# oleg-savchenko/jax_nbody_emulator_with_dj

Measured on AMD Instinct MI355X. Metric: voxels/sec (disp+vel) on 512^3 box, ndiv=4, higher is better.
Workload: dtype f32-equivalent: f16x3 split MFMA (3 f16 MFMAs per product, f32 accumulate)

## Files before the change

### jax_nbody_emulator_with_dj_amd/csrc/nbe_kernels_wino.h

```cpp

#ifndef NBE_EPI_MAX
#define NBE_EPI_MAX 1
#endif
#ifndef NBE_WINO_ZROW
#define NBE_WINO_ZROW 1
#endif
#ifndef NBE_WINO_ITEMREG
#define NBE_WINO_ITEMREG 1
#endif
#ifndef NBE_WINO_LOU
#define NBE_WINO_LOU (NBE_XF_F32 ? 0 : 1)
#endif
constexpr int NBE_MAX_WSTAGES = 32;
constexpr int NBE_MAX_WSKIP = 16;
constexpr float WINO_WSCALE = 16384.0f;
constexpr float WINO_WSCALE_F16 = 256.0f;

struct WinoSrc { const char* xa; const char* xb; long dxd; const char* w; long psb; float sb; int pad_; };

struct WinoKArgs {
    int H, W, Dv, Hv, Wv, Ho, Wo;
    int nchunk, cout_groups, flags, ntiles, tny, tnx;
    int zblock;
    float* y; float* dy; long out_pstride; int out_g0;
    const float* bias; const float* gout; const float* beta;
    const float* r; const float* dr; long res_pstride;
    float inv_scale;
    int nskip;
    long dws_delta;
    WinoSrc st[NBE_MAX_WSTAGES + NBE_MAX_WSKIP];
};

template <bool SKIP, bool NOVEL, bool F16 = false>
__global__ __launch_bounds__(512, 2) void conv_h3w_kernel(WinoKArgs a) {
    static_assert(!(F16 && NOVEL), "the float16 form has no displacement-only variant");
    typedef HGGeom<false> G;
    constexpr int NW = 8, CT = 64, TAPU = G::TAPU, WGU = G::WG, XBASE = G::XBASE, MT = 4, NT = 2, NTILE = 8;
    constexpr int ZROW = G::LDS_UNITS;
    f32x4* lds = lds_h3;
    const half8* L8 = (const half8*)lds_h3;
    half8* L8w = (half8*)lds_h3;
    const int tid = threadIdx.x;
    const int lane = tid & 63;
    const int wave = __builtin_amdgcn_readfirstlane(tid >> 6);
    const int c = lane & 15, q = lane >> 4, kh = q & 1, ks = q >> 1;

    const int nct = (a.cout_groups + 7) / 8;
    const int vt = xcd_tile(blockIdx.x, a.ntiles * nct);
    const int tile = vt / nct, ct = vt - tile * nct;
    const int npair = a.Dv >> 1;
    int zp, ty, tx;
    {
        const int zb = a.zblock;
        const int full = (npair / zb) * zb;
        const int per_blk = zb * a.tny * a.tnx;
        if (tile < (npair / zb) * per_blk) {
            const int blk = tile / per_blk, r = tile - blk * per_blk;
            const int zi = r % zb, tyx = r / zb;
            zp = blk * zb + zi; ty = tyx / a.tnx; tx = tyx - ty * a.tnx;
        } else {
            const int r = tile - (npair / zb) * per_blk, rem = npair - full;
            const int zi = r % rem, tyx = r / rem;
            zp = full + zi; ty = tyx / a.tnx; tx = tyx - ty * a.tnx;
        }
    }
    const int y0 = ty * (NOVEL ? 2 * HP_ROWS : HP_ROWS), x0 = tx * HP_COLS, z0 = 2 * zp;
    const int nst = 4 * a.nchunk;

    const long to = (((long)z0 * a.H + y0) * a.W + x0) * 16;
    const long wcm = (long)ct * nst * WGU * 16, wcs = (long)ct * a.nskip * TAPU * 16;

    struct Nxt { const char *xa, *xb, *w0; long dxd, psb; float sb; } nx;
    auto set_next = [&](int s) {
        const WinoSrc e = a.st[s];
        nx.xa = e.xa + to; nx.xb = e.xb + to; nx.dxd = e.dxd; nx.psb = e.psb; nx.w0 = e.w + (SKIP && s >= nst ? wcs : wcm); nx.sb = e.sb;
    };
    unsigned lane16 = (unsigned)lane << 4;
    asm volatile("" : "+v"(lane16));
    auto dma_w = [&](int buf, int t) {
        const int n = wave + NW * t;
        unsigned l16 = (unsigned)lane;
        if (NBE_WINO_ZROW && !F16) l16 = lane16;
        else asm volatile("v_lshlrev_b32 %0, 4, %0" : "+v"(l16));
        if (n < G::NWI) dma16s(nx.w0 + (long)n * 1024, l16, lds + buf * WGU + n * 64);
    };
    auto dma_raw = [&](int buf) {
        unsigned l16 = (unsigned)lane;
        asm volatile("v_lshlrev_b32 %0, 4, %0" : "+v"(l16));
        dma16s(nx.w0 + (wave < 4 ? 0 : a.dws_delta) + (long)(wave & 3) * 1024, l16, lds + buf * WGU + wave * 64);
#pragma unroll
        for (int t = 0; t < 6; ++t) {
            const int tensor = t / 3, n = wave + NW * (t % 3), pl = n / 6, k = n - 6 * pl;
            const int u = k * 64 + lane;
            const int uu = u < HP_PL ? u : HP_PL - 1;
            const int row = (uu * 241) >> 13, col = uu - row * HP_RS;
            if (u < HP_PL)
                dma16s(nx.xa + (tensor ? nx.dxd : 0) + (long)pl * nx.psb, (unsigned)(row * a.W + col) * 16u,
                       lds + XBASE + buf * HQ_XB + tensor * HQ_XT + pl * HQ_PP + k * 64);
        }
    };
    constexpr bool ITEMREG = NBE_WINO_ITEMREG && !F16;
    int it_uu[3] = {0, 0, 0};
    unsigned it_go[3] = {0u, 0u, 0u};
    if (ITEMREG) {
#pragma unroll
        for (int j = 0; j < 3; ++j) {
            const int u = ((wave + NW * j) % 6) * 64 + lane;
            it_uu[j] = u < HP_PL ? u : HP_PL - 1;
            const int row = (it_uu[j] * 241) >> 13, col = it_uu[j] - row * HP_RS;
            it_go[j] = (unsigned)(row * a.W + col) * 16u;
        }
#pragma unroll
        for (int j = 0; j < 3; ++j) asm volatile("" : "+v"(it_uu[j]), "+v"(it_go[j]));
    }
    auto item_unit = [&](int j, bool& valid) {
        if (ITEMREG) {
            valid = lane < HP_PL - ((wave + NW * j) % 6) * 64;
            return it_uu[j];
        }
        int l = lane;
        asm volatile("" : "+v"(l));
        const int u = ((wave + NW * j) % 6) * 64 + l;
        valid = u < HP_PL;
        return valid ? u : HP_PL - 1;
    };
    auto item_goff_j = [&](int j) {
        if (ITEMREG) return it_go[j];
        bool v;
        const int uu = item_unit(j, v);
        const int row = (uu * 241) >> 13, col = uu - row * HP_RS;
        return (unsigned)(row * a.W + col) * 16u;
    };
    typedef unsigned int u32x4 __attribute__((ext_vector_type(4)));
    struct Stg { half8 ah, al, bh, bl; float sb; };
    auto st_load = [&](int j, Stg& g) {
        const int n = wave + NW * j;
        const long po = ((n / 12) ? nx.dxd : 0) + (long)(((n % 12) / 6) * 2) * nx.psb;
        const char* pa = nx.xa + po;
        const char* pb = nx.xb + po;
        const unsigned go = item_goff_j(j);
        const __amdgpu_buffer_rsrc_t ra = __builtin_amdgcn_make_buffer_rsrc((void*)pa, 0, 0xffffffffu, 0x00027000);
        const __amdgpu_buffer_rsrc_t rb = __builtin_amdgcn_make_buffer_rsrc((void*)pb, 0, 0xffffffffu, 0x00027000);
        const unsigned pso = (unsigned)nx.psb;
        auto ld = [&](half8& d, __amdgpu_buffer_rsrc_t r, unsigned so) {
            const u32x4 v = __builtin_amdgcn_raw_buffer_load_b128(r, go, so, 0);
            d = __builtin_bit_cast(half8, v);
        };
        ld(g.ah, ra, 0); ld(g.al, ra, pso); ld(g.bh, rb, 0); ld(g.bl, rb, pso);
        g.sb = nx.sb;
    };
#if NBE_XF_F32
    struct Xf { u32x4 HI, LO; float t0, t1; unsigned h; };
    auto xf_step = [&](const Stg& g, Xf& x, int k) {
        const int r = k >> 2, m = k & 3;
        const unsigned AH = __builtin_bit_cast(u32x4, g.ah)[r], AL = __builtin_bit_cast(u32x4, g.al)[r];
        const unsigned BH = __builtin_bit_cast(u32x4, g.bh)[r], BL = __builtin_bit_cast(u32x4, g.bl)[r];
        const float inv = H3_INV, sinv = g.sb * H3_INV, sb = g.sb, k2048 = H3_SCALE;
        if (m == 0) {
            asm("v_fma_mix_f32 %0, %1, %2, %3 op_sel:[0,0,0] op_sel_hi:[1,0,1]" : "=v"(x.t0) : "v"(AL), "s"(inv), "v"(AH));
            asm("v_fma_mix_f32 %0, %1, %2, %0 op_sel:[0,0,0] op_sel_hi:[1,0,0]" : "+v"(x.t0) : "v"(BL), "s"(sinv));
            asm("v_fma_mix_f32 %0, %1, %2, %0 op_sel:[0,0,0] op_sel_hi:[1,0,0]" : "+v"(x.t0) : "v"(BH), "s"(sb));
        } else if (m == 1) {
            asm("v_fma_mix_f32 %0, %1, %2, %3 op_sel:[1,0,1] op_sel_hi:[1,0,1]" : "=v"(x.t1) : "v"(AL), "s"(inv), "v"(AH));
            asm("v_fma_mix_f32 %0, %1, %2, %0 op_sel:[1,0,0] op_sel_hi:[1,0,0]" : "+v"(x.t1) : "v"(BL), "s"(sinv));
            asm("v_fma_mix_f32 %0, %1, %2, %0 op_sel:[1,0,0] op_sel_hi:[1,0,0]" : "+v"(x.t1) : "v"(BH), "s"(sb));
        } else if (m == 2) {
            asm("v_cvt_pk_f16_f32 %0, %1, %2" : "=v"(x.h) : "v"(x.t0), "v"(x.t1));
            asm("v_fma_mix_f32 %0, %1, -1.0, %0 op_sel:[0,0,0] op_sel_hi:[1,0,0]" : "+v"(x.t0) : "v"(x.h));
            asm("v_fma_mix_f32 %0, %1, -1.0, %0 op_sel:[1,0,0] op_sel_hi:[1,0,0]" : "+v"(x.t1) : "v"(x.h));
        } else {
            unsigned l;
            asm("v_fma_mixlo_f16 %0, %1, %2, 0 op_sel_hi:[0,0,0]" : "=v"(l) : "v"(x.t0), "s"(k2048));
            asm("v_fma_mixhi_f16 %0, %1, %2, 0 op_sel_hi:[0,0,0]" : "+v"(l) : "v"(x.t1), "s"(k2048));
            x.HI[r] = x.h; x.LO[r] = l;
        }
    };
#else
    struct Xf { u32x4 HI, LO; unsigned s, bb, e1, e2, l1; };
    auto xf_step = [&](const Stg& g, Xf& x, int k) {
        const int r = k >> 2, m = k & 3;
        const unsigned AH = __builtin_bit_cast(u32x4, g.ah)[r], AL = __builtin_bit_cast(u32x4, g.al)[r];
        const unsigned BH = __builtin_bit_cast(u32x4, g.bh)[r], BL = __builtin_bit_cast(u32x4, g.bl)[r];
        const unsigned sbp = g.sb < 0.f ? 0xBC00BC00u : 0x3C003C00u, k2048 = 0x68006800u;
        if (F16) {
            if (m == 0) asm("v_pk_fma_f16 %0, %1, %2, %3" : "=v"(x.s) : "v"(BH), "s"(sbp), "v"(AH));
            else if (m == 1) asm("v_pk_fma_f16 %0, %1, %2, %3" : "=v"(x.l1) : "v"(BL), "s"(sbp), "v"(AL));
            else if (m == 3) { x.HI[r] = x.s; x.LO[r] = x.l1; }
            (void)k2048;
        } else
        if (m == 0) {
            asm("v_pk_fma_f16 %0, %1, %2, %3" : "=v"(x.s) : "v"(BH), "s"(sbp), "v"(AH));
            asm("v_pk_add_f16 %0, %1, %2 neg_lo:[0,1] neg_hi:[0,1]" : "=v"(x.bb) : "v"(x.s), "v"(AH));
        } else if (m == 1) {
            asm("v_pk_add_f16 %0, %1, %2 neg_lo:[0,1] neg_hi:[0,1]" : "=v"(x.e1) : "v"(x.s), "v"(x.bb));
            asm("v_pk_fma_f16 %0, %1, %2, %3 neg_lo:[0,0,1] neg_hi:[0,0,1]" : "=v"(x.e2) : "v"(BH), "s"(sbp), "v"(x.bb));
        } else if (m == 2) {
            asm("v_pk_add_f16 %0, %1, %2 neg_lo:[0,1] neg_hi:[0,1]" : "=v"(x.e1) : "v"(AH), "v"(x.e1));
            asm("v_pk_fma_f16 %0, %1, %2, %3" : "=v"(x.l1) : "v"(BL), "s"(sbp), "v"(AL));
        } else {
            unsigned err, l;
            asm("v_pk_add_f16 %0, %1, %2" : "=v"(err) : "v"(x.e1), "v"(x.e2));
#if NBE_WINO_LOU
            const unsigned kinv = 0x10001000u;
            asm("v_pk_fma_f16 %0, %1, %2, %3" : "=v"(l) : "v"(x.l1), "s"(kinv), "v"(err));
            (void)k2048;
#else
            asm("v_pk_fma_f16 %0, %1, %2, %3" : "=v"(l) : "v"(err), "s"(k2048), "v"(x.l1));
#endif
            x.HI[r] = x.s; x.LO[r] = l;
        }
    };
#endif
    auto st_write = [&](int j, int buf, const Xf& x) {
        bool valid;
        const int n = wave + NW * j;
        const int lo_ = XBASE + buf * HQ_XB + (n / 12) * HQ_XT + (((n % 12) / 6) * 2) * HQ_PP + item_unit(j, valid);
        if (valid) {
            L8w[lo_] = __builtin_bit_cast(half8, x.HI);
            L8w[lo_ + HQ_PP] = __builtin_bit_cast(half8, x.LO);
        }
    };
    auto st_store = [&](int j, int buf, Stg& g) {
        Xf x;
#pragma unroll
        for (int k = 0; k < 16; ++k) xf_step(g, x, k);
        st_write(j, buf, x);
    };

    f32x4 YA[NTILE], DA[NTILE], YB[NTILE], DB[NTILE];
#pragma unroll
    for (int t = 0; t < NTILE; ++t)
#pragma unroll
        for (int e = 0; e < 4; ++e) { YA[t][e] = 0.f; DA[t][e] = 0.f; YB[t][e] = 0.f; DB[t][e] = 0.f; }
    auto mm = [&](f32x4& acc, const half8& A, const half8& B) {
        asm("v_mfma_f32_16x16x32_f16 %0, %1, %2, %0" : "+a"(acc) : "v"(A), "v"(B));
    };
    auto mmz = [&](f32x4& acc, const half8& A, const half8& B) {
        asm("s_nop 1\n\tv_mfma_f32_16x16x32_f16 %0, %1, %2, %0" : "+a"(acc) : "v"(A), "v"(B));
    };

    const int rowp = wave;
    const int aP = (ks * 4 + 2 * kh) * CT + c;
    const int bB = (2 * kh) * HQ_PP + rowp * HP_RS + c;
    const int bP1 = bB + ks, bP32 = bB + 32 * ks;
    auto LA = [&](half8 (&r)[MT], int idx) {
#pragma unroll
        for (int mt = 0; mt < MT; ++mt) r[mt] = L8[idx + 16 * mt];
    };
    auto LB = [&](half8 (&r)[NT], int idx) {
#pragma unroll
        for (int nt = 0; nt < NT; ++nt) r[nt] = L8[idx + 16 * nt];
    };
    const _Float16 kInv = (_Float16)H3_INV;
#define SNAKE(i) ((((i) >> 1) & 1) ? ((i) ^ 1) : (i))
    auto nohook = [](int) {};
    auto MM8h = [&](f32x4 (&acc)[NTILE], const half8 (&A)[MT], const half8 (&B)[NT], int slot, int nb, bool px, bool zsel,
                    bool hooked, auto&& hook) {
#pragma unroll
        for (int i = 0; i < NTILE; ++i) {
            const int t = SNAKE(i);
            if (zsel && (i % NT) == 0) mmz(acc[t], A[t / NT], B[t % NT]); else
            mm(acc[t], A[t / NT], B[t % NT]);
            if (hooked) { hook(i); __builtin_amdgcn_sched_barrier(0); }
            if (slot >= 0 && (i % 4) == 3) {
                if (px) dma_w(nb, slot + i / 4);
                __builtin_amdgcn_sched_barrier(0);
            }
        }
    };
    auto MM8 = [&](f32x4 (&acc)[NTILE], const half8 (&A)[MT], const half8 (&B)[NT], int slot, int nb, bool px, bool zsel = false) {
        MM8h(acc, A, B, slot, nb, px, zsel, false, nohook);
    };
    auto MM8s = [&](f32x4 (&acc)[NTILE], half8 (&P)[MT], const half8 (&A)[MT], const half8 (&B)[NT], int slot, int nb, bool px) {
        P[0] = A[0] * kInv;
#pragma unroll
        for (int i = 0; i < NTILE; ++i) {
            const int t = SNAKE(i);
            if ((i % NT) == 0) { if (t / NT + 1 < MT) P[t / NT + 1] = A[t / NT + 1] * kInv; mmz(acc[t], P[t / NT], B[t % NT]); }
            else mm(acc[t], P[t / NT], B[t % NT]);
            if (slot >= 0 && (i % 4) == 3) {
                if (px) dma_w(nb, slot + i / 4);
                __builtin_amdgcn_sched_barrier(0);
            }
        }
    };
#define NBE_SB __builtin_amdgcn_sched_barrier(0)
    half8 wh[MT], wl[MT], wp[MT], xh[NT], xl[NT], dxh[NT], dxl[NT];
    auto pair = [&](f32x4 (&Y)[NTILE], f32x4 (&DY)[NTILE], int slot0, int nb, bool px, int wa, int xp,
                    auto&& preXl, auto&& preW, auto&& preXh, auto&& mid, bool hooked, auto&& hook, auto&& after3) {
        if (F16) {
            LB(dxh, xp + HQ_XT); LA(wl, wa + CT + aP);
            NBE_SB; MM8h(Y, wh, xh, slot0, nb, px, false, hooked, [&](int t) { hook(t); }); NBE_SB;
            LB(dxl, xp + HQ_XT + HQ_PP);
            NBE_SB; MM8h(Y, wl, xl, slot0 < 0 ? -1 : slot0 + 2, nb, px, false, hooked, [&](int t) { hook(8 + t); }); NBE_SB;
            after3();
            mid();
            preXl(); preXh();
            NBE_SB; MM8(DY, wh, dxh, slot0 < 0 ? -1 : slot0 + 4, nb, px); NBE_SB;
            preW();
            NBE_SB; MM8(DY, wl, dxl, -1, nb, px); NBE_SB;
            return;
        }
        LB(dxh, xp + HQ_XT);
#if NBE_WINO_LOU
        NBE_SB; MM8(Y, wh, xl, slot0, nb, px); NBE_SB;
#else
        NBE_SB; MM8s(Y, wp, wh, xl, slot0, nb, px); NBE_SB;
#endif
        LB(dxl, xp + HQ_XT + HQ_PP);
        NBE_SB; MM8h(Y, wh, xh, slot0 < 0 ? -1 : slot0 + 2, nb, px, false, hooked, [&](int t) { hook(t); }); NBE_SB;
        LA(wl, wa + CT + aP);
        NBE_SB; MM8h(DY, wh, dxh, slot0 < 0 ? -1 : slot0 + 4, nb, px, false, hooked, [&](int t) { hook(8 + t); }); NBE_SB;
        after3();
        mid();
#if NBE_WINO_LOU
        NBE_SB; MM8(DY, wh, dxl, -1, nb, px); NBE_SB;
#else
        NBE_SB; MM8(DY, wp, dxl, -1, nb, px); NBE_SB;
#endif
        preXl(); preW();
        NBE_SB; MM8(Y, wl, xh, -1, nb, px); NBE_SB;
        preXh();
        NBE_SB; MM8(DY, wl, dxh, -1, nb, px); NBE_SB;
    };

    constexpr int SH4 = HP_RS + 1, SH5 = HP_RS + 2, SH7 = 2 * HP_RS + 1;
    auto stage = [&](f32x4 (&Y)[NTILE], f32x4 (&DY)[NTILE], int s, auto nxt) {
        constexpr int NXT = decltype(nxt)::value;
        constexpr bool px = NXT == 1;
        const bool pre = px && s + 1 != 2 * a.nchunk;
        if (NXT) set_next(s + 1);
        int par = s & 1;
        asm volatile("" : "+s"(par));
        int nb = 1 - par;
        asm volatile("" : "+s"(nb));
        const int wb = par * WGU, xb = XBASE + par * HQ_XB;
        const int wbn = nb * WGU, xbn = XBASE + nb * HQ_XB;
        Stg g;
        Xf xf;
        auto hk = [&](int k) { xf_step(g, xf, k); };
        auto none = [] {};
        if (NXT == 2) dma_raw(nb);
        if (px) st_load(0, g);
        pair(Y, DY, 0, nb, px, wb, xb + bP1,
             [&] { LB(xl, xb + 2 + bP32 + HQ_PP); }, [&] { LA(wh, wb + 2 * TAPU + aP); }, [&] { LB(xh, xb + 2 + bP32); },
             none, false, nohook, none);
        half8 a1[MT], a2[MT], b1x[NT], b1d[NT];
        const int aS = wb + 4 * TAPU + (2 * kh + (F16 ? ks : 0)) * CT + c;
        const int bS = xb + (2 * kh + ks) * HQ_PP + rowp * HP_RS + c + SH4;
        pair(Y, DY, -1, nb, px, wb + 2 * TAPU, xb + 2 + bP32,
             [&] { LB(b1x, bS); }, [&] { LA(a1, aS); }, [&] { LB(b1d, bS + HQ_XT); }, none,
             px, hk, [&] { if (px) { st_write(0, nb, xf); st_load(1, g); } });
        const half8 zero = {0, 0, 0, 0, 0, 0, 0, 0};
        if (F16) {
            NBE_SB; MM8(Y, a1, b1x, -1, 0, false); NBE_SB;
            LB(xl, xb + SH5 + bP32 + HQ_PP); LB(xh, xb + SH5 + bP32); LA(wh, wb + 5 * TAPU + aP);
            NBE_SB; MM8(DY, a1, b1d, -1, 0, false); NBE_SB;
        } else {
#if NBE_WINO_LOU
        NBE_SB; MM8(Y, a1, b1x, -1, 0, false); NBE_SB;
#else
        {
            const _Float16 m1 = ks ? kInv : (_Float16)1.0f;
#pragma unroll
            for (int mt = 0; mt < MT; ++mt) a1[mt] = a1[mt] * m1;
        }
        NBE_SB; MM8(Y, a1, b1x, -1, 0, false, true); NBE_SB;
#endif
#if NBE_WINO_ZROW
        LA(a2, ks ? ZROW + c : aS + CT);
#else
        LA(a2, aS + CT);
#endif
        LB(xl, xb + SH5 + bP32 + HQ_PP);
        NBE_SB; MM8(DY, a1, b1d, -1, 0, false); NBE_SB;
        LB(xh, xb + SH5 + bP32); LA(wh, wb + 5 * TAPU + aP);
#if NBE_WINO_ZROW
        NBE_SB; MM8(Y, a2, b1x, -1, 0, false); NBE_SB;
#else
#pragma unroll
        for (int mt = 0; mt < MT; ++mt) a2[mt] = ks ? zero : a2[mt];
        NBE_SB; MM8(Y, a2, b1x, -1, 0, false, true); NBE_SB;
#endif
        MM8(DY, a2, b1d, -1, 0, false); NBE_SB;
        }
        pair(Y, DY, -1, nb, px, wb + 5 * TAPU, xb + SH5 + bP32,
             [&] { LB(xl, xb + SH7 + bP1 + HQ_PP); }, [&] { LA(wh, wb + 7 * TAPU + aP); }, [&] { LB(xh, xb + SH7 + bP1); },
             none, px, hk, [&] { if (px) { st_write(1, nb, xf); st_load(2, g); } });
        pair(Y, DY, -1, nb, px, wb + 7 * TAPU, xb + SH7 + bP1,
             [&] { if (pre) LB(xl, xbn + bP1 + HQ_PP); }, [&] { if (pre) LA(wh, wbn + aP); }, [&] { if (pre) LB(xh, xbn + bP1); },
             [&] { asm volatile("s_waitcnt vmcnt(0) lgkmcnt(0)\n\ts_barrier" ::: "memory"); },
             px, hk, [&] { if (px) st_write(2, nb, xf); });
    };

    auto raw_stage = [&](f32x4 (&Y)[NTILE], f32x4 (&DY)[NTILE], int s, bool px) {
        if (px) set_next(s + 1);
        int par = s & 1;
        asm volatile("" : "+s"(par));
        int nb = 1 - par;
        asm volatile("" : "+s"(nb));
        const int wb = par * WGU, xb = XBASE + par * HQ_XB;
        if (px) dma_raw(nb);
        half8 a1[MT], a2[MT], d1[MT], d2[MT], bx[NT], bd[NT];
        const half8 zero = {0, 0, 0, 0, 0, 0, 0, 0};
        const _Float16 m1 = ks ? kInv : (_Float16)1.0f;
        const int aS = wb + (2 * kh) * CT + c;
        const int bS = xb + (2 * kh + ks) * HQ_PP + rowp * HP_RS + c + SH4;
        if (F16) {
            const int aF = wb + (2 * kh + ks) * CT + c;
            LA(a1, aF); LB(bx, bS); LB(bd, bS + HQ_XT); LA(d1, aF + TAPU);
            NBE_SB; MM8(Y, a1, bx, -1, 0, false); NBE_SB;
            MM8(DY, a1, bd, -1, 0, false); NBE_SB;
            MM8(DY, d1, bx, -1, 0, false); NBE_SB;
            asm volatile("s_waitcnt vmcnt(0) lgkmcnt(0)\n\ts_barrier" ::: "memory");
            return;
        }
        LA(a1, aS); LB(bx, bS); LA(a2, aS + CT); LB(bd, bS + HQ_XT);
#pragma unroll
        for (int mt = 0; mt < MT; ++mt) a1[mt] = a1[mt] * m1;
        NBE_SB; MM8(Y, a1, bx, -1, 0, false, true); NBE_SB;
        if (!NOVEL) LA(d1, aS + TAPU);
#pragma unroll
        for (int mt = 0; mt < MT; ++mt) a2[mt] = ks ? zero : a2[mt];
        NBE_SB; MM8(Y, a2, bx, -1, 0, false, true); NBE_SB;
        if (!NOVEL) LA(d2, aS + TAPU + CT);
        if (NOVEL || !(a.flags & F_SKIP_NODX)) {
            NBE_SB; MM8(DY, a1, bd, -1, 0, false); NBE_SB;
            MM8(DY, a2, bd, -1, 0, false); NBE_SB;
        }
        if (!NOVEL) {
#pragma unroll
            for (int mt = 0; mt < MT; ++mt) { d1[mt] = d1[mt] * m1; d2[mt] = ks ? zero : d2[mt]; }
            NBE_SB; MM8(DY, d1, bx, -1, 0, false, true); NBE_SB;
            MM8(DY, d2, bx, -1, 0, false, true); NBE_SB;
        }
        asm volatile("s_waitcnt vmcnt(0) lgkmcnt(0)\n\ts_barrier" ::: "memory");
    };

    {
        if (NBE_WINO_ZROW && !F16 && tid < 64) L8w[ZROW + tid] = half8{0, 0, 0, 0, 0, 0, 0, 0};
        set_next(0);
#pragma unroll
        for (int k = 0; k < G::NWS; ++k) dma_w(0, k);
        {
            Stg g0, g1, g2;
            st_load(0, g0); st_load(1, g1); st_load(2, g2);
            st_store(0, 0, g0); st_store(1, 0, g1); st_store(2, 0, g2);
        }
        asm volatile("s_waitcnt vmcnt(0) lgkmcnt(0)" ::: "memory");
        __syncthreads();
        LA(wh, aP); LB(xl, XBASE + bP1 + HQ_PP); LB(xh, XBASE + bP1);
    }

    auto butterfly = [&] {
            asm volatile("s_nop 15\n\ts_nop 15" ::: "memory");
#pragma unroll
            for (int t = 0; t < NTILE; ++t) {
                f32x4 p, m;
#pragma unroll
                for (int e = 0; e < 4; ++e) { p[e] = acc_read(YA[t][e]); m[e] = acc_read(YB[t][e]); }
                YA[t] = p + m; YB[t] = p - m;
                asm volatile("" : "+a"(YA[t]), "+a"(YB[t]));
                __builtin_amdgcn_sched_barrier(0);
#pragma unroll
                for (int e = 0; e < 4; ++e) { p[e] = acc_read(DA[t][e]); m[e] = acc_read(DB[t][e]); }
                DA[t] = p + m; DB[t] = p - m;
                asm volatile("" : "+a"(DA[t]), "+a"(DB[t]));
                __builtin_amdgcn_sched_barrier(0);
            }
            asm volatile("s_nop 7" ::: "memory");
            LA(wh, aP); LB(xl, XBASE + bP1 + HQ_PP); LB(xh, XBASE + bP1);
    };
    const int npairs = 2 * a.nchunk;
    for (int s2 = 0; s2 + 1 < npairs; ++s2) {
        if (s2 == a.nchunk) butterfly();
        stage(YA, DA, 2 * s2, std::integral_constant<int, 1>());
        stage(YB, DB, 2 * s2 + 1, std::integral_constant<int, 1>());
    }
    if (npairs - 1 == a.nchunk) butterfly();
    stage(YA, DA, 2 * npairs - 2, std::integral_constant<int, 1>());
    stage(YB, DB, 2 * npairs - 1, std::integral_constant<int, SKIP ? 2 : 0>());
    if (SKIP) {
        for (int sc = 0; sc < a.nskip; ++sc) {
            raw_stage(YA, DA, nst + 2 * sc, true);
            raw_stage(YB, DB, nst + 2 * sc + 1, sc + 1 < a.nskip);
        }
    }
#undef NBE_SB
#undef SNAKE
    asm volatile("s_nop 15\n\ts_nop 15" ::: "memory");

    const bool act = a.flags & F_ACT, gauge = !NOVEL && a.gout != nullptr;
    f32x4 bv[MT], be[MT], gv[MT];
    int unit[MT];
    bool uok[MT];
#pragma unroll
    for (int mt = 0; mt < MT; ++mt) {
        unit[mt] = ct * (CT / 8) + 2 * mt + ks;
        uok[mt] = unit[mt] < a.cout_groups;
        if (!uok[mt]) unit[mt] = a.cout_groups - 1;
        bv[mt] = *(const f32x4*)(a.bias + unit[mt] * 8 + 4 * kh);
        be[mt] = f32x4{0.f, 0.f, 0.f, 0.f};
        if (!NOVEL) be[mt] = *(const f32x4*)(a.beta + unit[mt] * 8 + 4 * kh);
        gv[mt] = f32x4{0.f, 0.f, 0.f, 0.f};
        if (!NOVEL && gauge) gv[mt] = *(const f32x4*)(a.gout + unit[mt] * 8 + 4 * kh);
    }
#pragma unroll
    for (int mt = 0; mt < MT; ++mt) asm volatile("" : "+v"(bv[mt]), "+v"(be[mt]), "+v"(gv[mt]));
    long ob_mt[MT];
#pragma unroll
    for (int mt = 0; mt < MT; ++mt) ob_mt[mt] = (long)(a.out_g0 + (F16 ? 1 : 2) * unit[mt]) * a.out_pstride * 16 + 8 * kh;
    const long ol_off = a.out_pstride * 16;
    auto epilogue = [&](f32x4 (&Y)[NTILE], f32x4 (&DY)[NTILE], int z) {
        int o[NT];
        bool ook[NT], ook2[NT];
#pragma unroll
        for (int nt = 0; nt < NT; ++nt) {
            const int yy = y0 + rowp, xx = x0 + 16 * nt + c;
            ook[nt] = yy < a.Hv && xx < a.Wv;
            ook2[nt] = NOVEL && yy + HP_ROWS < a.Hv && xx < a.Wv;
            o[nt] = ook[nt] ? (z * a.Ho + yy) * a.Wo + xx : z * a.Ho * a.Wo;
        }
        half4 r0[F16 ? NTILE : 1], r1[F16 ? NTILE : 1];
        const bool res = F16 && (a.flags & F_RES);
        if (F16 && res) {
#pragma unroll
            for (int t = 0; t < NTILE; ++t) {
                const int mt = t / NT, nt = t % NT;
                const long rb = ((long)unit[mt] * a.res_pstride + (long)o[nt]) * 16 + 8 * kh;
                r0[t] = *(const half4*)((const char*)a.r + rb);
                r1[t] = *(const half4*)((const char*)a.dr + rb);
            }
#pragma unroll
            for (int t = 0; t < NTILE; ++t) asm volatile("" : "+v"(r0[t]), "+v"(r1[t]));
        }
#pragma unroll
        for (int mt = 0; mt < MT; ++mt) {
#pragma unroll
            for (int nt = 0; nt < NT; ++nt) {
                const int t = mt * NT + nt;
                f32x4 v, dv;
                __builtin_amdgcn_sched_barrier(0);
#pragma unroll
                for (int e = 0; e < 4; ++e) {
                    const float yp = acc_read(Y[t][e]) * a.inv_scale;
                    v[e] = yp + bv[mt][e];
                    dv[e] = acc_read(DY[t][e]) * a.inv_scale + be[mt][e] * yp;
                }
                if (F16 && res) {
#pragma unroll
                    for (int e = 0; e < 4; ++e) { v[e] += (float)r0[t][e]; dv[e] += (float)r1[t][e]; }
                }
                if (act) {
#pragma unroll
                    for (int e = 0; e < 4; ++e) {
                        dv[e] = v[e] > 0.f ? dv[e] : 0.01f * dv[e];
                        v[e] = (F16 || !NBE_EPI_MAX) ? (v[e] >= 0.f ? v[e] : 0.01f * v[e]) : __builtin_fmaxf(v[e], 0.01f * v[e]);
                    }
                }
                if (gauge) {
#pragma unroll
                    for (int e = 0; e < 4; ++e) dv[e] += gv[mt][e] * v[e];
                }
                if (F16) {
                    if (uok[mt] && ook[nt]) {
                        const long ob = ob_mt[mt] + (long)o[nt] * 16;
                        half4 h, dh;
#pragma unroll
                        for (int e = 0; e < 4; ++e) { h[e] = (_Float16)v[e]; dh[e] = (_Float16)dv[e]; }
                        *(half4*)((char*)a.y + ob) = h;
                        *(half4*)((char*)a.dy + ob) = dh;
                    }
                } else
                if (NOVEL) {
#pragma unroll
                    for (int e = 0; e < 4; ++e) {
                        dv[e] = acc_read(DY[t][e]) * a.inv_scale + bv[mt][e];
                        if (act) dv[e] = dv[e] >= 0.f ? dv[e] : 0.01f * dv[e];
                    }
                    const long ob = ob_mt[mt] + (long)o[nt] * 16;
                    const long ol = ob + ol_off;
                    const long r8 = (long)HP_ROWS * a.Wo * 16;
                    half4 hi, lo;
                    if (uok[mt] && ook[nt]) {
                        split4(v, hi, lo);
                        *(half4*)((char*)a.y + ob) = hi;
                        *(half4*)((char*)a.y + ol) = lo;
                    }
                    if (uok[mt] && ook2[nt]) {
                        split4(dv, hi, lo);
                        *(half4*)((char*)a.y + ob + r8) = hi;
                        *(half4*)((char*)a.y + ol + r8) = lo;
                    }
                } else
                if (uok[mt] && ook[nt]) {
                    const long ob = ob_mt[mt] + (long)o[nt] * 16;
                    const long ol = ob + ol_off;
                    half4 hi, lo;
                    split4(v, hi, lo);
                    *(half4*)((char*)a.y + ob) = hi;
                    *(half4*)((char*)a.y + ol) = lo;
                    split4(dv, hi, lo);
                    *(half4*)((char*)a.dy + ob) = hi;
                    *(half4*)((char*)a.dy + ol) = lo;
                }
            }
        }
    };
    epilogue(YA, DA, z0);
    epilogue(YB, DB, z0 + 1);
}

__global__ __launch_bounds__(256) void pack_h3w_kernel(const float* __restrict__ w, int cout, int cin, int nchunk, long total,
                                                       _Float16* __restrict__ dst, int* __restrict__ flag, int f16) {
    const long idx = (long)blockIdx.x * blockDim.x + threadIdx.x;
    if (idx >= total) return;
    long r = idx;
    const int j = (int)(r % 8); r /= 8;
    const int co = (int)(r % 64); r /= 64;
    const int u = (int)(r % 4); r /= 4;
    const int tap = (int)(r % 9); r /= 9;
    const int stage = (int)(r % (4 * nchunk)); r /= 4 * nchunk;
    const int ct = (int)r;
    const int chunk = stage >> 2, xi = stage & 3;
    const int h = u >> 1, part = u & 1;
    const int ci = f16 ? chunk * 32 + 8 * u + j : chunk * 16 + 8 * h + j, oc = ct * 64 + co;
    float v = 0.f;
    if (oc < cout && ci < cin) {
        const float* p = w + (((size_t)oc * cin + ci) * 3) * 9 + tap;
        const float w0 = p[0], w1 = p[9], w2 = p[18];
        v = xi == 0 ? w0 : xi == 1 ? 0.5f * (w0 + w1 + w2) : xi == 2 ? 0.5f * (w0 - w1 + w2) : -w2;
    }
    v *= f16 ? WINO_WSCALE_F16 : WINO_WSCALE;
    if (!(fabsf(v) <= 60000.f)) { atomicOr(flag, 1); v = 0.f; }
    const _Float16 hi = (_Float16)v;
    dst[idx] = (part == 0 || f16) ? hi : (_Float16)(v - (float)hi);
}

void launch_pack_h3w(const float* w_oidhw, int cout, int cin, int cin_pad, int ctiles, float* dst, int* flag, hipStream_t s, int prec) {
    const bool f16 = prec == PREC_F16;
    const int nchunk = cin_pad / (f16 ? 32 : 16);
    const long total = (long)ctiles * 4 * nchunk * 9 * 4 * 64 * 8;
    hipLaunchKernelGGL(pack_h3w_kernel, dim3((unsigned)((total + 255) / 256)), dim3(256), 0, s, w_oidhw, cout, cin, nchunk, total,
                       (_Float16*)dst, flag, f16 ? 1 : 0);
}

static int launch_h3w(const ConvKArgs& ka_in, const float* ww, const float* wws, long wws_set_floats, int ctiles, hipStream_t s,
                      bool novel = false, bool f16 = false) {
    typedef HGGeom<false> G;
    constexpr size_t smem = (size_t)(G::LDS_UNITS + 64) * 16;
    static_assert(smem <= 160 * 1024, "LDS budget of one CU");
    ConvKArgs ka = ka_in;
    if (f16) {
        if (novel || (ka.nchunk & 1) || (ka.csplit < ka.nchunk && (ka.csplit & 1))) return 1;
        if (ka.nskip > 0 && ((ka.nskip & 1) || (ka.s_csplit < ka.nskip && (ka.s_csplit & 1)) || (ka.flags & F_SKIP_NODX))) return 1;
        ka.nchunk /= 2; if (ka.csplit < (1 << 29)) ka.csplit /= 2;
        ka.nskip /= 2; if (ka.s_csplit < (1 << 29)) ka.s_csplit /= 2;
    }
    if (!ww || (!f16 && (ka.flags & F_RES)) || (ka.Dv & 1) || 4 * ka.nchunk > NBE_MAX_WSTAGES || (!novel && !ka.beta)) return 1;
    if (ka.nskip > 0 && (!wws || 2 * ka.nskip > NBE_MAX_WSKIP)) return 1;
    if (ctiles != (ka.cout_groups + 7) / 8) return 1;
    if (std::max(ka.in_pstride, ka.csplit < ka.nchunk ? ka.in2_pstride : 0L) * 16 + 16L * (HP_ROWS + 2) * ka.W >= (1L << 32) - (1L << 20)) return 1;
    WinoKArgs wa;
    wa.H = ka.H; wa.W = ka.W; wa.Dv = ka.Dv; wa.Hv = ka.Hv; wa.Wv = ka.Wv; wa.Ho = ka.Ho; wa.Wo = ka.Wo;
    wa.nchunk = ka.nchunk; wa.cout_groups = ka.cout_groups; wa.flags = ka.flags;
    const int trows = novel ? 2 * HP_ROWS : HP_ROWS;
    wa.tny = (ka.Hv + trows - 1) / trows;
    wa.tnx = (ka.Wv + HP_COLS - 1) / HP_COLS;
    wa.ntiles = (ka.Dv / 2) * wa.tny * wa.tnx;
    wa.y = ka.y; wa.dy = ka.dy; wa.out_pstride = ka.out_pstride; wa.out_g0 = ka.out_g0;
    wa.bias = ka.bias; wa.gout = novel ? nullptr : ka.gout; wa.beta = novel ? nullptr : ka.beta;
    const long rows8 = (long)HP_ROWS * ka.W * 16;
    wa.inv_scale = 1.0f / (f16 ? WINO_WSCALE_F16 : WINO_WSCALE);
    wa.r = ka.r; wa.dr = ka.dr; wa.res_pstride = ka.res_pstride;
    wa.zblock = std::min(8, ka.Dv / 2);
    wa.nskip = ka.nskip; wa.dws_delta = wws_set_floats * 4;
    static const int XI[2][2] = {{1, 2}, {0, 3}};
    static const int PA[4] = {0, 1, 2, 1}, PB[4] = {2, 2, 1, 3};
    static const float SB[4] = {-1.f, 1.f, -1.f, -1.f};
    const long plane = (long)ka.H * ka.W * 16;
    for (int ph = 0; ph < 2; ++ph)
        for (int chunk = 0; chunk < ka.nchunk; ++chunk)
            for (int ab = 0; ab < 2; ++ab) {
                const int xi = XI[ph][ab];
                const bool second = chunk >= ka.csplit;
                const long ps = second ? ka.in2_pstride : ka.in_pstride;
                const char* x = (const char*)(second ? ka.x2 : ka.x);
                const char* dx = (const char*)(second ? ka.dx2 : ka.dx);
                const long off = (long)(second ? chunk - ka.csplit : chunk) * 4 * ps * 16;
                WinoSrc& e = wa.st[(ph * ka.nchunk + chunk) * 2 + ab];
                e.xa = x + off + PA[xi] * plane; e.xb = x + off + PB[xi] * plane; e.dxd = novel ? rows8 : dx - x;
                e.w = (const char*)ww + (long)(chunk * 4 + xi) * G::WG * 16; e.psb = ps * 16; e.sb = SB[xi]; e.pad_ = 0;
            }
    for (int sc = 0; sc < ka.nskip; ++sc)
        for (int ab = 0; ab < 2; ++ab) {
            const bool second = sc >= ka.s_csplit;
            const long ps = second ? ka.s2_pstride : ka.s_pstride;
            const char* x = (const char*)(second ? ka.xs2 : ka.xs);
            const char* dx = (const char*)(second ? ka.dxs2 : ka.dxs);
            const long off = (long)(second ? sc - ka.s_csplit : sc) * 4 * ps * 16 + ab * plane;
            WinoSrc& e = wa.st[4 * ka.nchunk + 2 * sc + ab];
            e.xa = x + off; e.xb = e.xa; e.dxd = novel ? rows8 : dx - x; e.w = (const char*)wws + (long)sc * G::TAPU * 16; e.psb = ps * 16; e.sb = 0.f; e.pad_ = 0;
        }
    const bool skip = ka.nskip > 0;
    if (novel) wa.dws_delta = 0;
    auto kern = f16 ? (skip ? conv_h3w_kernel<true, false, true> : conv_h3w_kernel<false, false, true>)
              : novel ? (skip ? conv_h3w_kernel<true, true> : conv_h3w_kernel<false, true>)
              : (skip ? conv_h3w_kernel<true, false> : conv_h3w_kernel<false, false>);
    ensure_lds_limit((const void*)kern, smem);
    dim3 grid(wa.ntiles * ctiles, 1, 1), block(512, 1, 1);
    hipLaunchKernelGGL(kern, grid, block, smem, s, wa);
    return 0;
}
```

Measured before the change: 97.89 million.

## Preload all skip weights to LDS and stream skip activations via registers

For the non-F16 skip path, the kernel now DMAs every skip chunk's weights into the idle LDS buffers in one go at the last main stage. Skip-input activations are loaded straight from global memory into registers with double buffering, replacing the per-stage LDS staging and its barriers. The skip loop is restructured into raw_chunk, which processes YA and YB in the same pass and folds the scale into MFMA hooks. This aims to remove the per-skip-stage barrier and DMA round trips, but adds register pressure and global-load latency exposure, and limits the number of skip chunks to eight.

```diff
diff --git a/jax_nbody_emulator_with_dj_amd/csrc/nbe_kernels_wino.h b/jax_nbody_emulator_with_dj_amd/csrc/nbe_kernels_wino.h
--- a/jax_nbody_emulator_with_dj_amd/csrc/nbe_kernels_wino.h
+++ b/jax_nbody_emulator_with_dj_amd/csrc/nbe_kernels_wino.h
@@ -68,12 +68,17 @@
     const int nst = 4 * a.nchunk;
 
     const long to = (((long)z0 * a.H + y0) * a.W + x0) * 16;
-    const long wcm = (long)ct * nst * WGU * 16, wcs = (long)ct * a.nskip * TAPU * 16;
+    const long wcm = (long)ct * nst * WGU * 16;
+    auto wcs_of = [&] { return (long)ct * a.nskip * TAPU * 16; };
 
     struct Nxt { const char *xa, *xb, *w0; long dxd, psb; float sb; } nx;
     auto set_next = [&](int s) {
         const WinoSrc e = a.st[s];
-        nx.xa = e.xa + to; nx.xb = e.xb + to; nx.dxd = e.dxd; nx.psb = e.psb; nx.w0 = e.w + (SKIP && s >= nst ? wcs : wcm); nx.sb = e.sb;
+        nx.xa = e.xa + to; nx.xb = e.xb + to; nx.dxd = e.dxd; nx.psb = e.psb; nx.w0 = e.w + wcm; nx.sb = e.sb;
+    };
+    auto set_next_raw = [&](int s) {
+        const WinoSrc e = a.st[s];
+        nx.xa = e.xa + to; nx.xb = e.xb + to; nx.dxd = e.dxd; nx.psb = e.psb; nx.w0 = e.w + wcs_of(); nx.sb = e.sb;
     };
     unsigned lane16 = (unsigned)lane << 4;
     asm volatile("" : "+v"(lane16));
@@ -98,6 +103,16 @@
                 dma16s(nx.xa + (tensor ? nx.dxd : 0) + (long)pl * nx.psb, (unsigned)(row * a.W + col) * 16u,
                        lds + XBASE + buf * HQ_XB + tensor * HQ_XT + pl * HQ_PP + k * 64);
         }
+    };
+    constexpr int SKWU = 2 * TAPU;
+    static_assert(4 * SKWU <= WGU && 4 * SKWU <= HQ_XB && 2 * 8 <= NBE_MAX_WSKIP, "eight chunks of skip weights fit the idle buffers");
+    auto skw = [&](int buf, int sc) { return sc < 4 ? buf * WGU + sc * SKWU : XBASE + buf * HQ_XB + (sc - 4) * SKWU; };
+    auto dma_skipw = [&](int buf) {
+        unsigned l16 = (unsigned)lane;
+        asm volatile("v_lshlrev_b32 %0, 4, %0" : "+v"(l16));
+#pragma nounroll
+        for (int sc = 0; sc < a.nskip; ++sc)
+            dma16s(a.st[nst + 2 * sc].w + wcs_of() + (wave < 4 ? 0 : a.dws_delta) + (long)(wave & 3) * 1024, l16, lds + skw(buf, sc) + wave * 64);
     };
     constexpr bool ITEMREG = NBE_WINO_ITEMREG && !F16;
     int it_uu[3] = {0, 0, 0};
@@ -324,12 +339,34 @@
         NBE_SB; MM8(DY, wl, dxh, -1, nb, px); NBE_SB;
     };
 
+    struct RawB { half8 x[2][NT], d[2][NT]; };
+    RawB rb0, rb1;
+    const bool skdx = NOVEL || !(a.flags & F_SKIP_NODX);
+    auto raw_load = [&](int sc, RawB& b, bool on) {
+        int l = lane;
+        asm volatile("" : "+v"(l));
+        const unsigned vox = (unsigned)((wave + 1) * a.W + 1 + (l & 15)) * 16u;
+        const unsigned pl = (unsigned)(2 * ((l >> 4) & 1) + (l >> 5));
+#pragma unroll
+        for (int ab = 0; ab < 2; ++ab) {
+            const WinoSrc& e = a.st[nst + 2 * sc + ab];
+            const char* gx = e.xa + to + (on ? (long)pl * e.psb + vox : 0L);
+            const char* gd = gx + (skdx ? e.dxd : 0L);
+#pragma unroll
+            for (int nt = 0; nt < NT; ++nt) {
+                b.x[ab][nt] = *(const half8*)(gx + 256 * nt);
+                b.d[ab][nt] = *(const half8*)(gd + 256 * nt);
+            }
+        }
+    };
+
     constexpr int SH4 = HP_RS + 1, SH5 = HP_RS + 2, SH7 = 2 * HP_RS + 1;
     auto stage = [&](f32x4 (&Y)[NTILE], f32x4 (&DY)[NTILE], int s, auto nxt) {
         constexpr int NXT = decltype(nxt)::value;
         constexpr bool px = NXT == 1;
         const bool pre = px && s + 1 != 2 * a.nchunk;
-        if (NXT) set_next(s + 1);
+        if (NXT == 1) set_next(s + 1);
+        if (NXT == 2 && F16) set_next_raw(s + 1);
         int par = s & 1;
         asm volatile("" : "+s"(par));
         int nb = 1 - par;
@@ -340,7 +377,10 @@
         Xf xf;
         auto hk = [&](int k) { xf_step(g, xf, k); };
         auto none = [] {};
-        if (NXT == 2) dma_raw(nb);
+        if (NXT == 2) {
+            if (F16) dma_raw(nb);
+            else { dma_skipw(nb); raw_load(0, rb0, true); }
+        }
         if (px) st_load(0, g);
         pair(Y, DY, 0, nb, px, wb, xb + bP1,
              [&] { LB(xl, xb + 2 + bP32 + HQ_PP); }, [&] { LA(wh, wb + 2 * TAPU + aP); }, [&] { LB(xh, xb + 2 + bP32); },
@@ -389,56 +429,77 @@
              none, px, hk, [&] { if (px) { st_write(1, nb, xf); st_load(2, g); } });
         pair(Y, DY, -1, nb, px, wb + 7 * TAPU, xb + SH7 + bP1,
              [&] { if (pre) LB(xl, xbn + bP1 + HQ_PP); }, [&] { if (pre) LA(wh, wbn + aP); }, [&] { if (pre) LB(xh, xbn + bP1); },
-             [&] { asm volatile("s_waitcnt vmcnt(0) lgkmcnt(0)\n\ts_barrier" ::: "memory"); },
+             [&] {
+                 if (NXT == 2 && !F16) {
+                     __builtin_amdgcn_s_waitcnt(0x0070);
+                     asm volatile("s_barrier" ::: "memory");
+                 } else
+                 asm volatile("s_waitcnt vmcnt(0) lgkmcnt(0)\n\ts_barrier" ::: "memory");
+             },
              px, hk, [&] { if (px) st_write(2, nb, xf); });
     };
 
     auto raw_stage = [&](f32x4 (&Y)[NTILE], f32x4 (&DY)[NTILE], int s, bool px) {
-        if (px) set_next(s + 1);
+        if (px) set_next_raw(s + 1);
         int par = s & 1;
         asm volatile("" : "+s"(par));
         int nb = 1 - par;
         asm volatile("" : "+s"(nb));
         const int wb = par * WGU, xb = XBASE + par * HQ_XB;
         if (px) dma_raw(nb);
-        half8 a1[MT], a2[MT], d1[MT], d2[MT], bx[NT], bd[NT];
-        const half8 zero = {0, 0, 0, 0, 0, 0, 0, 0};
-        const _Float16 m1 = ks ? kInv : (_Float16)1.0f;
-        const int aS = wb + (2 * kh) * CT + c;
+        half8 a1[MT], d1[MT], bx[NT], bd[NT];
         const int bS = xb + (2 * kh + ks) * HQ_PP + rowp * HP_RS + c + SH4;
-        if (F16) {
-            const int aF = wb + (2 * kh + ks) * CT + c;
-            LA(a1, aF); LB(bx, bS); LB(bd, bS + HQ_XT); LA(d1, aF + TAPU);
-            NBE_SB; MM8(Y, a1, bx, -1, 0, false); NBE_SB;
-            MM8(DY, a1, bd, -1, 0, false); NBE_SB;
-            MM8(DY, d1, bx, -1, 0, false); NBE_SB;
-            asm volatile("s_waitcnt vmcnt(0) lgkmcnt(0)\n\ts_barrier" ::: "memory");
-            return;
-        }
-        LA(a1, aS); LB(bx, bS); LA(a2, aS + CT); LB(bd, bS + HQ_XT);
-#pragma unroll
-        for (int mt = 0; mt < MT; ++mt) a1[mt] = a1[mt] * m1;
-        NBE_SB; MM8(Y, a1, bx, -1, 0, false, true); NBE_SB;
-        if (!NOVEL) LA(d1, aS + TAPU);
-#pragma unroll
-        for (int mt = 0; mt < MT; ++mt) a2[mt] = ks ? zero : a2[mt];
-        NBE_SB; MM8(Y, a2, bx, -1, 0, false, true); NBE_SB;
-        if (!NOVEL) LA(d2, aS + TAPU + CT);
-        if (NOVEL || !(a.flags & F_SKIP_NODX)) {
-            NBE_SB; MM8(DY, a1, bd, -1, 0, false); NBE_SB;
-            MM8(DY, a2, bd, -1, 0, false); NBE_SB;
+        const int aF = wb + (2 * kh + ks) * CT + c;
+        LA(a1, aF); LB(bx, bS); LB(bd, bS + HQ_XT); LA(d1, aF + TAPU);
+        NBE_SB; MM8(Y, a1, bx, -1, 0, false); NBE_SB;
+        MM8(DY, a1, bd, -1, 0, false); NBE_SB;
+        MM8(DY, d1, bx, -1, 0, false); NBE_SB;
+        asm volatile("s_waitcnt vmcnt(0) lgkmcnt(0)\n\ts_barrier" ::: "memory");
+    };
+
+    const int skb = nst & 1;
+    auto raw_A = [&](half8 (&r)[MT], int sc, int which) {
+        int wS = skw(skb, sc);
+        asm volatile("" : "+s"(wS));
+        const int hi = wS + (which >> 1) * TAPU + (2 * kh) * CT + c;
+        LA(r, (which & 1) ? (ks ? ZROW + c : hi + CT) : hi);
+    };
+    const _Float16 km1 = ks ? kInv : (_Float16)1.0f;
+    auto raw_scale = [&](half8 (&r)[MT], int i) {
+#pragma unroll
+        for (int e = 0; e < 4; ++e) r[i >> 1][4 * (i & 1) + e] = r[i >> 1][4 * (i & 1) + e] * km1;
+    };
+    auto raw_chunk = [&](int sc, RawB& cur, RawB& nxt, half8 (&P)[MT], half8 (&Q)[MT]) {
+        const bool more = sc + 1 < a.nskip;
+        const int sn = more ? sc + 1 : sc;
+        raw_load(sn, nxt, more);
+        auto scaleP = [&](int i) { raw_scale(P, i); };
+        NBE_SB; MM8(YA, P, cur.x[0], -1, 0, false); NBE_SB;
+        MM8(YB, P, cur.x[1], -1, 0, false); NBE_SB;
+        if (skdx) {
+            MM8(DA, P, cur.d[0], -1, 0, false); NBE_SB;
+            MM8(DB, P, cur.d[1], -1, 0, false); NBE_SB;
+        }
+        raw_A(P, NOVEL ? sn : sc, NOVEL ? 0 : 2);
+        NBE_SB; MM8(YA, Q, cur.x[0], -1, 0, false); NBE_SB;
+        MM8h(YB, Q, cur.x[1], -1, 0, false, false, true, scaleP); NBE_SB;
+        if (skdx) {
+            MM8(DA, Q, cur.d[0], -1, 0, false); NBE_SB;
+            MM8(DB, Q, cur.d[1], -1, 0, false); NBE_SB;
         }
         if (!NOVEL) {
-#pragma unroll
-            for (int mt = 0; mt < MT; ++mt) { d1[mt] = d1[mt] * m1; d2[mt] = ks ? zero : d2[mt]; }
-            NBE_SB; MM8(DY, d1, bx, -1, 0, false, true); NBE_SB;
-            MM8(DY, d2, bx, -1, 0, false, true); NBE_SB;
-        }
-        asm volatile("s_waitcnt vmcnt(0) lgkmcnt(0)\n\ts_barrier" ::: "memory");
+            raw_A(Q, sc, 3);
+            NBE_SB; MM8(DA, P, cur.x[0], -1, 0, false); NBE_SB;
+            MM8(DB, P, cur.x[1], -1, 0, false); NBE_SB;
+            raw_A(P, sn, 0);
+            NBE_SB; MM8(DA, Q, cur.x[0], -1, 0, false); NBE_SB;
+            MM8h(DB, Q, cur.x[1], -1, 0, false, false, true, scaleP); NBE_SB;
+        }
+        raw_A(Q, sn, 1);
     };
 
     {
-        if (NBE_WINO_ZROW && !F16 && tid < 64) L8w[ZROW + tid] = half8{0, 0, 0, 0, 0, 0, 0, 0};
+        if ((NBE_WINO_ZROW || SKIP) && !F16 && tid < 64) L8w[ZROW + tid] = half8{0, 0, 0, 0, 0, 0, 0, 0};
         set_next(0);
 #pragma unroll
         for (int k = 0; k < G::NWS; ++k) dma_w(0, k);
@@ -480,10 +541,22 @@
     if (npairs - 1 == a.nchunk) butterfly();
     stage(YA, DA, 2 * npairs - 2, std::integral_constant<int, 1>());
     stage(YB, DB, 2 * npairs - 1, std::integral_constant<int, SKIP ? 2 : 0>());
-    if (SKIP) {
+    if (SKIP && F16) {
         for (int sc = 0; sc < a.nskip; ++sc) {
             raw_stage(YA, DA, nst + 2 * sc, true);
             raw_stage(YB, DB, nst + 2 * sc + 1, sc + 1 < a.nskip);
+        }
+    }
+    if (SKIP && !F16) {
+        half8 P[MT], Q[MT];
+        raw_A(P, 0, 0);
+#pragma unroll
+        for (int i = 0; i < 8; ++i) raw_scale(P, i);
+        raw_A(Q, 0, 1);
+        asm volatile("s_nop 1" : "+v"(P[0]), "+v"(P[1]), "+v"(P[2]), "+v"(P[3]));
+        for (int sc = 0; sc < a.nskip; sc += 2) {
+            raw_chunk(sc, rb0, rb1, P, Q);
+            if (sc + 1 < a.nskip) raw_chunk(sc + 1, rb1, rb0, P, Q);
         }
     }
 #undef NBE_SB
```

Measured after the change: 99.04 million (median of 6 runs). 1.01x the previous value.
